# mconati/armour-dev

Hardware: AMD Instinct MI355X
Metric: planning iterations/sec (7-DOF, 100 t-steps, 20 obs) (higher is better)
Workload: dtype f64; 1 GPU; Kinova Gen3 7-DOF, T=100, O=20 box obstacles, 3 concurrent planner(s) x 1308 worlds/GPU/step; obstacles=20, worlds_per_gpu=3924, planners_per_gpu=3, worlds_per_planner=1308, parallelism=world-sharded x1, RCCL all_gather of per-world records

## Files before the change

### armour-dev_amd/armour_amd/__init__.py

```python
from __future__ import annotations

import ctypes
import os

import numpy as np

from .robots import KINOVA
from .worlds import csv_world, example_world, make_world, straight_line_waypoint

_HERE = os.path.dirname(os.path.abspath(__file__))
LIB_PATH = os.environ.get("ARMOUR_LIB") or os.path.join(_HERE, "libarmour_hip.so")
NF = 7
_LIB = None
_dp = ctypes.POINTER(ctypes.c_double)


ARMOUR_E_ARG, ARMOUR_E_HIP, ARMOUR_E_CAPACITY, ARMOUR_E_STATE, ARMOUR_E_INTERNAL = -1, -2, -3, -4, -5


class ArmourError(RuntimeError):
    pass


class Config(ctypes.Structure):
# ... 607 lines not shown
        lk = np.zeros((self.T, self.NJ), dtype=np.int32)
        tq = np.zeros((self.T, NF), dtype=np.int32)
        _check(lib().armour_get_monomial_counts(self.h, w, lk.ctypes.data_as(ctypes.POINTER(ctypes.c_int)),
                                                tq.ctypes.data_as(ctypes.POINTER(ctypes.c_int))))
        return lk, tq

    OCCUPANCY = ("arena_hashes", "arena_rows", "operator_terms", "link_monomials", "torque_monomials",
                 "worlds_retried", "worlds_failed")

    def occupancy(self):
        n = len(self.OCCUPANCY)
        used = (ctypes.c_longlong * n)()
        caps = (ctypes.c_longlong * n)()
        rc = lib().armour_get_reach_occupancy(self.h, used, caps, n)
        _check(min(0, rc))
        return {k: (int(used[i]), int(caps[i])) for i, k in enumerate(self.OCCUPANCY)}

    def reach_span_ms(self):
        v = ctypes.c_double()
        _check(lib().armour_get_reach_span(self.h, ctypes.byref(v)))
        return v.value

    def plane_cache_stats(self):
        keys = ("planes_kept", "pairs", "blocks_cached", "blocks", "max_per_pair", "pool_records", "box_misses")
        out = (ctypes.c_longlong * len(keys))()
        _check(min(0, lib().armour_get_plane_cache_stats(self.h, out, len(keys))))
        return {k: int(out[i]) for i, k in enumerate(keys)}

    def torque_radius(self, w):
        r = np.zeros((self.T, NF))
        _check(lib().armour_get_torque_radius(self.h, w, _ptr(r)))
        return r


def run_episodes(planner, worlds, goals, max_steps, track=None, **config):
    st = planner.episode_begin(worlds, goals, **config)
    if track is not None:
        planner.episode_track(**track)
    running = int(np.sum(st["status"] == 0))
    for _ in range(int(max_steps)):
        if running == 0:
            break
        running, _, _ = planner.episode_step()
    st = planner.episode_states()
    out = dict(status=st["status"], steps=st["steps"], clearance=st["clearance"])
    if track is not None:
        out["tracked"] = planner.episode_tracked()
# ... 39 lines not shown
```

### armour-dev_amd/csrc/nlp.h

```cpp
#pragma once
#include "reach.h"

namespace armour {

constexpr int EVAL_THREADS = 256;
constexpr int ROW_THREADS = 256;
constexpr int MAX_FILTER = 64;
constexpr int KA = 56;
constexpr int KA2 = 8;

struct IpmOpts {
    double tol = 1e-4;
    int max_iter = 100;
    double mu0 = 0.1;
    double kappa_eps = 10.0;
    double kappa_mu = 0.2;
    double theta_mu = 1.5;
    double tau_min = 0.99;
    double bound_push = 1e-2;
    double eta = 1e-4;
    int max_ls = 10;
    double kappa_sigma = 1e10;
    double s_max = 100.0;
    double inf_bound = 1e19;
// ... 56 lines not shown
    WorldState* ws;
    int* flags;
    const int* wl;
    int* wl_run;
    int* wl_search;
    unsigned* cnt;
    int ls0;
    const unsigned* lcount;
    unsigned* lcount_out;
    unsigned* lrun_out;
    int* nrun_flag;
    int* bt_flag;
    int K;
    double *gs, *fs, *partial_s;
    int b_in_cs;
    int resto;
    int rflag;
    int* rl_app;
    int* pend_flag;
    int pcache;
    int pcready;
    long pc_pool;
    double* pc;
    uint16_t* pcp;
    unsigned* pcoff;
    unsigned char* pcok;
    unsigned long long* pcbase;
    unsigned* pcnext;
    const int* Ow;
};
constexpr int EV_MAXK = 9;
constexpr int PC_K = 12;
constexpr double PC_XBOX = 1.0 + 1e-6;
constexpr double PC_RADF = 1.0001;
constexpr double PC_MARGIN = 1e-9;

AD int world_of(const NlpDev& d, int b) { return d.wl ? d.wl[b] : b; }

AD long gidx(const NlpDev& d, int slot, int w, long r) { return ((long)slot * d.W + w) * d.m + r; }

struct Shape {
    int O, m, R, nblk;
};
template <bool MX>
AD Shape shape_of(const NlpDev& d, int w) {
    if constexpr (MX) {
        const int O = d.Ow[w];
        const int m = d.nt + d.T * d.NJ * O + 4 * NF;
        const int R = m + NF;
        return Shape{O, m, R, (R + d.chunk - 1) / d.chunk};
    } else {
        return Shape{d.O, d.m, d.R, d.nblk};
    }
}

// ... 2 lines not shown
```

### armour-dev_amd/csrc/nlp_kernels.hip

```cpp
#include "nlp.h"

namespace armour {

__device__ inline double wave_max(double v) {
#pragma unroll
    for (int m = 1; m < 64; m <<= 1) v = fmax(v, xor_f64(v, m));
    return v;
}
__device__ inline double wave_min(double v) {
#pragma unroll
    for (int m = 1; m < 64; m <<= 1) v = fmin(v, xor_f64(v, m));
    return v;
}
template <int N>
__device__ inline void block_reduce_n(double (&v)[N], const int (&kinds)[N], double* lds, double* out) {
    const int wave = threadIdx.x >> 6, nw = blockDim.x >> 6;
#pragma unroll
    for (int g = 0; g < N; g += 8) {
#pragma unroll
        for (int i = g; i < (g + 8 < N ? g + 8 : N); i++)
            v[i] = kinds[i] == 0 ? wave_sum(v[i]) : kinds[i] == 1 ? wave_max(v[i]) : wave_min(v[i]);
        if ((threadIdx.x & 63) == 0) {
#pragma unroll
            for (int i = g; i < (g + 8 < N ? g + 8 : N); i++) lds[wave * N + i] = v[i];
// ... 346 lines not shown
    const unsigned long long u = __builtin_bit_cast(unsigned long long, x);
    return (u >> 63) ? ~u : (u | 0x8000000000000000ull);
}
__device__ inline double dkey(unsigned long long k) {
    return __builtin_bit_cast(double, (k >> 63) ? (k & 0x7FFFFFFFFFFFFFFFull) : ~k);
}

template <bool MX>
__device__ __attribute__((always_inline)) void plane_cache_body(const NlpDev& d) {
    const int t = blockIdx.x, w = blockIdx.y, tid = threadIdx.x;
    const long jt = (long)w * d.T + t;
    const int NJ = d.NJ, O = shape_of<MX>(d, w).O, NP = NJ * O;
    const int OS = d.O, NPS = NJ * OS;
    __shared__ double cen[MAX_J][3], rad[MAX_J][3];
    __shared__ double lgen[MAX_J][18];
    __shared__ double obs[MAX_OBS][12];
    __shared__ double llp[MAX_J][LL_PLANES][10];
    __shared__ double oop[MAX_OBS][OO_PLANES][5];
    __shared__ double mixlo[MAX_J * MAX_OBS * OBS_GEN];
    __shared__ unsigned char mixbits[MAX_J * MAX_OBS * OBS_GEN];
    __shared__ double pairM[MAX_J * MAX_OBS];
    __shared__ unsigned cntp[MAX_J * MAX_OBS];
    __shared__ unsigned long long pbits[MAX_J * MAX_OBS];
    __shared__ unsigned total_s;
    for (int i = tid; i < NJ * 18; i += blockDim.x) lgen[i / 18][i % 18] = d.ro.link_gens[jt * NJ * 18 + i];
    for (int i = tid; i < O * 12; i += blockDim.x) obs[i / 12][i % 12] = d.obs[(long)w * OS * 12 + i];
    if (tid < NJ * 3) {
        const int l = tid / 3, e = tid % 3;
        const long b = jt * NJ + l;
        const int cnt = d.ro.link_cnt[b];
        double r = 0.0;
        for (int q = 0; q < cnt; q++) r += fabs(d.ro.link_coef[(b * CAP_LM + q) * 3 + e]);
        cen[l][e] = d.ro.link_center[b * 3 + e];
        rad[l][e] = r * PC_RADF;
    }
    __syncthreads();
    for (int u = tid; u < NJ * LL_PLANES + O * OO_PLANES; u += blockDim.x) {
        if (u < NJ * LL_PLANES) ll_table(lgen[u / LL_PLANES], u % LL_PLANES, cen[u / LL_PLANES], llp[u / LL_PLANES][u % LL_PLANES]);
        else oo_table(obs[(u - NJ * LL_PLANES) / OO_PLANES], (u - NJ * LL_PLANES) % OO_PLANES,
                      oop[(u - NJ * LL_PLANES) / OO_PLANES][(u - NJ * LL_PLANES) % OO_PLANES]);
    }
    const int nmix = NP * OBS_GEN;
    auto load_gens = [&](int l, int o, double (*G)[3], double* oc) {
#pragma unroll
        for (int r = 0; r < 3; r++) oc[r] = obs[o][r];
#pragma unroll
        for (int q = 0; q < OBS_GEN; q++)
#pragma unroll
            for (int r = 0; r < 3; r++) G[q][r] = obs[o][(q + 1) * 3 + r];
#pragma unroll
        for (int q = 0; q < 6; q++)
#pragma unroll
            for (int r = 0; r < 3; r++) G[OBS_GEN + q][r] = lgen[l][r + 3 * q];
    };
    __syncthreads();
    for (int u = tid; u < nmix; u += blockDim.x) {
        const int l = u / (O * OBS_GEN), o = (u / OBS_GEN) % O, i = u % OBS_GEN;
        double G[BUF_GEN][3], oc[3];
        load_gens(l, o, G, oc);
        double M = -1e300;
        const double* const ga = obs[o] + 3 * (i + 1);
#pragma unroll
        for (int j = 0; j < 6; j++) {
            double A[3], dd, del, lo, hi;
            mixed_plane_j(j, ga, G, oc, A, dd, del);
            pc_bounds(A, dd + del, -dd + del, cen[l], rad[l], lo, hi);
            if (nonzero3(A)) M = fmax(M, lo);
        }
        mixlo[u] = M;
    }
    __syncthreads();
    for (int pr = tid; pr < NP; pr += blockDim.x) {
        const int l = pr / O, o = pr % O;
        double G[BUF_GEN][3], oc[3];
        load_gens(l, o, G, oc);
        double M = fmax(fmax(mixlo[pr * 3], mixlo[pr * 3 + 1]), mixlo[pr * 3 + 2]);
#pragma unroll
        for (int p = 0; p < OO_PLANES; p++) {
// ... 21 lines not shown
#pragma unroll
        for (int j = 0; j < 6; j++) {
            double A[3], dd, del, lo, hi;
            mixed_plane_j(j, ga, G, oc, A, dd, del);
            pc_bounds(A, dd + del, -dd + del, cen[l], rad[l], lo, hi);
            if (nonzero3(A) && hi >= M) bits |= 1u << j;
        }
        mixbits[u] = (unsigned char)bits;
    }
    __syncthreads();
    auto survives = [&](int pr, int l, int o, int a, int b, const double (*G)[3], const double* oc) -> bool {
        if (a < OBS_GEN && b >= OBS_GEN) return (mixbits[pr * OBS_GEN + a] >> (b - OBS_GEN)) & 1;
        const double* P = b < OBS_GEN ? oop[o][a + b - 1] : llp[l][(a - OBS_GEN) * (11 - (a - OBS_GEN)) / 2 + b - a - 1];
        double dd, del, lo, hi;
        if (b < OBS_GEN) oo_complete(P, G + OBS_GEN, dd, del);
        else ll_complete(P, G, oc, dd, del);
        pc_bounds(P, dd + del, -dd + del, cen[l], rad[l], lo, hi);
        return nonzero3(P) && hi >= pairM[pr] - PC_MARGIN;
    };
    for (int pr = tid; pr < NP; pr += blockDim.x) {
        const int l = pr / O, o = pr % O;
        double G[BUF_GEN][3], oc[3];
        load_gens(l, o, G, oc);
        unsigned n = 0;
        unsigned long long bits = 0;
        int pos = 0;
        for (int a = 0; a < BUF_GEN; a++)
            for (int b = a + 1; b < BUF_GEN; b++, pos++)
                if (survives(pr, l, o, a, b, G, oc)) {
                    n++;
                    bits |= 1ull << pos;
                }
        cntp[pr] = n;
        pbits[pr] = bits;
    }
    __syncthreads();
    if (tid < 64) {
        const int per = (NP + 63) / 64, b0 = tid * per;
        unsigned s = 0;
        for (int q = b0; q < b0 + per && q < NP; q++) s += cntp[q];
        unsigned incl = s;
#pragma unroll
        for (int off = 1; off < 64; off <<= 1) {
            const unsigned v = __shfl_up(incl, off);
            if (tid >= off) incl += v;
        }
        unsigned run = incl - s;
        for (int q = b0; q < b0 + per && q < NP; q++) {
            const unsigned c = cntp[q];
            cntp[q] = run;
            run += c;
            d.pcoff[jt * NPS + q] = (run - c) << 8 | c;
        }
        if (tid == 63) total_s = incl;
    }
    __syncthreads();
    __shared__ unsigned long long base_s;
    if (tid == 0) {
        const unsigned long long b0 = atomicAdd(d.pcnext, total_s);
        const bool fits = b0 + total_s <= (unsigned long long)d.pc_pool;
        d.pcok[jt] = fits ? 1 : 0;
        d.pcbase[jt] = fits ? b0 : 0;
        base_s = fits ? b0 : ~0ull;
    }
    __syncthreads();
    if (base_s == ~0ull) return;
    double* const rec = d.pc + 5 * base_s;
    uint16_t* const pcp = d.pcp + base_s;
    const int cap = (int)total_s;
    for (int pr = tid; pr < NP; pr += blockDim.x) {
        const int l = pr / O, o = pr % O;
        double G[BUF_GEN][3], oc[3];
        load_gens(l, o, G, oc);
        unsigned q = cntp[pr];
        const unsigned long long bits = pbits[pr];
        int pos = 0;
        for (int a = 0; a < BUF_GEN; a++)
            for (int b = a + 1; b < BUF_GEN; b++) {
                if (!((bits >> pos++) & 1ull)) continue;
                double A[3], dd, del;
                if (a < OBS_GEN && b >= OBS_GEN) {
                    mixed_plane_j(b - OBS_GEN, obs[o] + 3 * (a + 1), G, oc, A, dd, del);
                } else {
                    const double* P = b < OBS_GEN ? oop[o][a + b - 1] : llp[l][(a - OBS_GEN) * (11 - (a - OBS_GEN)) / 2 + b - a - 1];
                    A[0] = P[0]; A[1] = P[1]; A[2] = P[2];
                    if (b < OBS_GEN) oo_complete(P, G + OBS_GEN, dd, del);
                    else ll_complete(P, G, oc, dd, del);
                }
                rec[q] = A[0];
                rec[cap + q] = A[1];
                rec[2 * cap + q] = A[2];
                rec[3 * cap + q] = dd + del;
                rec[4 * cap + q] = -dd + del;
                pcp[q] = (uint16_t)pr;
                q++;
            }
    }
}
__global__ __launch_bounds__(EVAL_THREADS) void plane_cache_kernel(NlpDev d) { plane_cache_body<false>(d); }
__global__ __launch_bounds__(EVAL_THREADS) void plane_cache_kernel_mx(NlpDev d) { plane_cache_body<true>(d); }


#define STAGE_MONOMIALS_BODY                                                                        \
    int lpre[MAX_J + 1], tpre[NF + 1];                                                              \
    lpre[0] = 0;                                                                                    \
    _Pragma("unroll") for (int l = 0; l < MAX_J; l++) lpre[l + 1] = lpre[l] + (l < NJ ? lcnt[l] : 0); \
    tpre[0] = 0;                                                                                    \
    _Pragma("unroll") for (int j = 0; j < NF; j++) tpre[j + 1] = tpre[j] + tcnt[j];                 \
    const int L = lpre[MAX_J], M = tpre[NF];                                                        \
    for (int u = threadIdx.x; u < L + M; u += blockDim.x) {                                         \
        if (u < L) {                                                                                \
            int l = 0, q0 = 0;                                                                      \
            _Pragma("unroll") for (int k = 1; k < MAX_J; k++) if (u >= lpre[k]) { l = k; q0 = lpre[k]; } \
            const int q = u - q0;                                                                   \
            const long b = (jt * NJ + l) * CAP_LM + q;                                              \
            lh[l][q] = d.ro.link_hash[b];                                                           \
            lco[l][q][0] = d.ro.link_coef[b * 3];                                                   \
// ... 62 lines not shown
    return r;
}
#define TRAJ_COST_BODY                                                                              \
    for (int j = 0; j < NF; j++)                                                                    \
        qp[j] = bz_q(ts.q0[j], ts.qd0[j] * ts.D, ts.qdd0[j] * ts.D * ts.D, rp.k_range[j] * x[j], tp); \
    double fv = 0.0;                                                                                \
    bool first = true;                                                                              \
    for (int pass = 1; pass >= 0; pass--)                                                           \
        for (int j = 0; j < NF; j++) {                                                              \
            if (rp.wrap_mask[j] != pass) continue;                                                  \
            const double dd = pass ? wrap_to_pi(d.qdes[w * NF + j] - qp[j]) : (d.qdes[w * NF + j] - qp[j]); \
            const double term = dd * dd;                                                            \
            fv = first ? term : fv + term;                                                          \
            first = false;                                                                          \
        }
__device__ __attribute__((always_inline)) double traj_cost(const NlpDev& d, const RobotParams& rp, TrajStart ts, int w,
                                                           const double* x, double* qp) {
    const double tp = rp.t_plan;
    TRAJ_COST_BODY
    return fv;
}

struct PlaneRecords {
    const double* rec;
    const uint16_t* pcp;
    int total;
};
__device__ __attribute__((always_inline)) PlaneRecords plane_records(const NlpDev& d, long jt, int NP, bool some = true) {
    const unsigned last = some ? d.pcoff[jt * (d.NJ * d.O) + NP - 1] : 0u;
    const unsigned long long pb = d.pcbase[jt];
    return {d.pc + 5 * pb, d.pcp + pb, (int)(last >> 8) + (int)(last & 255)};
}
struct PlaneRecord {
    double a[3], P, N;
    int pr;
};
__device__ __attribute__((always_inline)) PlaneRecord load_record(PlaneRecords pc, int q) {
    const int cap = pc.total;
    return {{pc.rec[q], pc.rec[cap + q], pc.rec[2 * cap + q]}, pc.rec[3 * cap + q], pc.rec[4 * cap + q], pc.pcp[q]};
}
__device__ __attribute__((always_inline)) double record_candidate(PlaneRecord r, const double* lc, bool& neg) {
    const double Ac = r.a[0] * lc[0] + r.a[1] * lc[1] + r.a[2] * lc[2];
    const double pos = Ac - r.P, nv = -Ac - r.N;
    neg = nv > pos || pos != pos;
    return neg ? nv : pos;
}
constexpr double SCAN_START = -100000000.0;
__device__ __attribute__((always_inline)) void pair_max(unsigned long long* key, double v) {
    if (v > SCAN_START) atomicMax(key, okey(v));
}

constexpr int UB_FULL = MAX_J * CAP_LM * 3 + NF * CAP_UM;
constexpr int LM_S = 16, UM_S = 64;
constexpr int UB_S = 1544;
static_assert(UB_S >= MAX_J * LM_S * 3 + NF * UM_S, "small staging buffer");
__host__ __device__ constexpr int eval_pair_doubles(int np) { return np + (np + 1) / 2 + 4 * np; }
template <typename R, bool ARMTD, bool CACHED, int LM, int UM, int UB, bool MX = false>
__device__ __attribute__((always_inline)) void eval_body(const NlpDev& d, int mode) {
    static_assert(!CACHED || std::is_same<R, double>::value, "the plane cache is fp64");
    static_assert(!MX || (std::is_same<R, double>::value && !ARMTD), "mixed batches: the fp64 ARMOUR planner");
    if ((mode == 1 || mode == 5) && d.lcount && blockIdx.y >= *d.lcount) return;
    const int t = blockIdx.x, w = world_of(d, blockIdx.y);
    WorldState& S = d.ws[w];
// ... 25 lines not shown
    auto lco = reinterpret_cast<R (*)[LM][3]>(ubuf);
    auto tco = reinterpret_cast<R (*)[UM]>(ubuf + MAX_J * LM * 3);
    constexpr int NMIX = MAX_J * MAX_OBS * OBS_GEN;
    static_assert(CACHED || MAX_J * LL_PLANES * 10 + MAX_OBS * OO_PLANES * 5 + NMIX + (NMIX + 7) / 8 <= UB, "plane tables");
    auto llp = reinterpret_cast<R (*)[LL_PLANES][10]>(ubuf);
    auto oop = reinterpret_cast<R (*)[OO_PLANES][5]>(ubuf + MAX_J * LL_PLANES * 10);
    R* mixv = reinterpret_cast<R*>(ubuf + MAX_J * LL_PLANES * 10 + MAX_OBS * OO_PLANES * 5);
    int8_t* mixc = reinterpret_cast<int8_t*>(mixv + NMIX);
    __shared__ int lcnt[MAX_J], tcnt[NF];
    __shared__ R ptab[NF][8];
    if (tid < NF) {
        const double xd = mode == 0 ? S.x[tid] : S.xt[tid];
        x[tid] = xd;
        const R xj = (R)xd;
        power_table(xj, ptab[tid]);
        ptab[tid][4] = (R)0.0; ptab[tid][5] = (R)1.0 * (R)1.0; ptab[tid][6] = (R)2.0 * xj; ptab[tid][7] = (R)3.0 * (xj * xj);
    }
    if (tid < NJ) lcnt[tid] = d.ro.link_cnt[jt * NJ + tid];
    if (tid >= 32 && tid < 32 + NF) tcnt[tid - 32] = d.nt ? d.ro.tq_cnt[jt * NF + tid - 32] : 0;
    if constexpr (!CACHED) {
        for (int i = tid; i < NJ * 18; i += blockDim.x) lgen[i / 18][i % 18] = d.ro.link_gens[jt * NJ * 18 + i];
        for (int i = tid; i < O * 12; i += blockDim.x) obs[i / 12][i % 12] = d.obs[(long)w * OS * 12 + i];
    }
    __syncthreads();
    EVP_MARK
    if (!(d.diag & 1)) {
        STAGE_MONOMIALS_BODY
    }
    __syncthreads();
    EVP_MARK
    const int nlk = NJ * 3 * 8;
    for (int u = tid; u < ((d.diag & 1) ? 0 : 64 + nlk); u += blockDim.x) {
      if (u >= 64) {
        const int ul = u - 64;
        const int l = ul / 24, e = (ul / 8) % 3, k = ul % 8;
        const long base = jt * NJ + l;
        R c = k == 0 ? d.ro.link_center[base * 3 + e] : 0.0;
        c = sum4(c, lcnt[l], [&](int q) { return slice_term(lco[l][q][e], lh[l][q], k, ptab); });
        if (k == 0) {
            const R r = d.ro.link_rad[base * 3 + e];
            const R cc = interval_mid(c, r);
            lc[l][e] = cc;
            Lcb[((long)t * NJ + l) * 3 + e] = cc;
        } else {
            dlc[l][k - 1][e] = c;
            Jdb[(((long)t * NJ + l) * NF + k - 1) * 3 + e] = c;
// ... 39 lines not shown
            *fb = fv * rp.cost_scale;
            for (int i = 0; i < NF; i++) {
                const double dk = tp * tp * tp * (6 * tp * tp - 15 * tp + 10) * rp.k_range[i];
                double gv = rp.wrap_mask[i] ? (2 * wrap_to_pi(qp[i] - d.qdes[w * NF + i]) * dk) : (2 * (qp[i] - d.qdes[w * NF + i]) * dk);
                gradb[i] = gv * rp.cost_scale;
            }
        }
    }
    __syncthreads();
    EVP_MARK
    const long nt = d.nt;
    bool coll = !(d.diag & 2);
    if constexpr (MX) coll = coll && O > 0;
    if constexpr (CACHED) {
        bool inbox = true;
#pragma unroll
        for (int j = 0; j < NF; j++) inbox = inbox && fabs(x[j]) <= PC_XBOX;
        if (coll && !inbox) {
            for (int pr = tid; pr < NJ * O; pr += blockDim.x)
                Gb[nt + ((long)(pr / O) * d.T + t) * O + pr % O] = __builtin_nan("");
            if (tid == 0) atomicAdd(d.cnt + 7, 1u);
        } else if (coll) {
            const int NP = NJ * O;
            const PlaneRecords pc = plane_records(d, jt, NP);
            const int total = pc.total;
            unsigned long long* const pkey = reinterpret_cast<unsigned long long*>(ubuf);
            unsigned* const pidx = reinterpret_cast<unsigned*>(ubuf + NP);
            double* const pB = ubuf + NP + (NP + 1) / 2;
            static_assert(eval_pair_doubles(MAX_J * MAX_OBS) <= UB_FULL, "pair tables");
            const double start = SCAN_START;
            for (int pr = tid; pr < NP; pr += blockDim.x) {
                pkey[pr] = okey(start);
                pidx[pr] = 0xFFFFFFFFu;
            }
            __syncthreads();
            EVP_MARK
            auto cand = [&](int q, double& v, int& sub, int& pr, double* a) {
                const PlaneRecord r = load_record(pc, q);
                a[0] = r.a[0]; a[1] = r.a[1]; a[2] = r.a[2];
                pr = r.pr;
                bool neg;
                v = record_candidate(r, lc[pr / O], neg);
                sub = neg ? 1 : 0;
            };
            constexpr int RPT = 3;
            if (total <= RPT * EVAL_THREADS) {
                double v[RPT], a[RPT][3];
                int sub[RPT], pq[RPT];
#pragma unroll
                for (int s = 0; s < RPT; s++) {
                    const int q = tid + s * EVAL_THREADS;
                    v[s] = start;
                    sub[s] = 0;
                    pq[s] = 0;
                    if (q < total) {
                        cand(q, v[s], sub[s], pq[s], a[s]);
                        pair_max(&pkey[pq[s]], v[s]);
                    }
                }
                __syncthreads();
                EVP_MARK
#pragma unroll
                for (int s = 0; s < RPT; s++) {
                    const int q = tid + s * EVAL_THREADS;
                    if (q < total && v[s] > start && v[s] == dkey(pkey[pq[s]])) atomicMin(&pidx[pq[s]], (unsigned)(2 * q + sub[s]));
                }
                __syncthreads();
                EVP_MARK
#pragma unroll
                for (int s = 0; s < RPT; s++) {
                    const int q = tid + s * EVAL_THREADS;
                    if (q < total && pidx[pq[s]] == (unsigned)(2 * q + sub[s])) {
                        double* const b = pB + pq[s] * 4;
                        b[0] = a[s][0]; b[1] = a[s][1]; b[2] = a[s][2]; b[3] = v[s];
                    }
                }
            } else {
                for (int q = tid; q < total; q += blockDim.x) {
                    double v, a[3];
                    int sub, pr;
                    cand(q, v, sub, pr, a);
                    pair_max(&pkey[pr], v);
                }
                __syncthreads();
                EVP_MARK
                for (int q = tid; q < total; q += blockDim.x) {
                    double v, a[3];
                    int sub, pr;
                    cand(q, v, sub, pr, a);
                    if (v > start && v == dkey(pkey[pr])) atomicMin(&pidx[pr], (unsigned)(2 * q + sub));
                }
                __syncthreads();
                EVP_MARK
                for (int q = tid; q < total; q += blockDim.x) {
                    double v, a[3];
                    int sub, pr;
                    cand(q, v, sub, pr, a);
                    if (pidx[pr] == (unsigned)(2 * q + sub)) {
                        double* const b = pB + pr * 4;
                        b[0] = a[0]; b[1] = a[1]; b[2] = a[2]; b[3] = v;
                    }
                }
            }
            __syncthreads();
            EVP_MARK
            for (int pr = tid; pr < NP; pr += blockDim.x) {
                const int l = pr / O, o = pr % O;
                const unsigned wi = pidx[pr];
                const bool won = wi != 0xFFFFFFFFu, isneg = won && (wi & 1u);
                const double* const b = pB + pr * 4;
                const double best = won ? b[3] : start;
                const double B0 = won ? b[0] : 0.0, B1 = won ? b[1] : 0.0, B2 = won ? b[2] : 0.0;
                const long row = nt + ((long)l * d.T + t) * O + o;
                Gb[row] = -best;
                double* const jn = Jnb + (row - nt) * 3;
                jn[0] = isneg ? B0 : -B0;
                jn[1] = isneg ? B1 : -B1;
                jn[2] = isneg ? B2 : -B2;
                if (mode == 0) {
#pragma unroll
                    for (int kk = 0; kk < NF; kk++) {
                        const double dot = B0 * dlc[l][kk][0] + B1 * dlc[l][kk][1] + B2 * dlc[l][kk][2];
                        Jb[row * NF + kk] = isneg ? dot : -dot;
                    }
                }
            }
            coll = false;
        }
    }
    if constexpr (!CACHED) {
    for (int u = tid; u < (coll ? NJ * LL_PLANES + O * OO_PLANES : 0); u += blockDim.x) {
        if (u < NJ * LL_PLANES) {
            const int l = u / LL_PLANES, p = u % LL_PLANES;
            ll_table(lgen[l], p, lc[l], llp[l][p]);
        } else {
// ... 193 lines not shown
            const double c = sum4(d.ro.tq_center[base], tcnt[j], [&](int q) { return value_term(tco[j][q], th[j][q], ptab[kk]); });
            d.gs[((long)i * K + kk) * d.m + (long)t * NF + j] = interval_mid(c, d.ro.tq_rad[base]);
        }
    }
    for (int v = t; v <= 2 * NF && tid >= (int)blockDim.x - K; v += d.T) {
        const int kk = tid - ((int)blockDim.x - K);
        const double* x = xk[kk];
        double* const Gb = d.gs + ((long)i * K + kk) * d.m;
        const TrajStart ts = traj_start(d, w);
        if (v < 2 * NF) {
            const long off2 = (long)NF * d.T + (long)d.T * d.NJ * O;
            const int kind = v / NF, j = v % NF;
            const ExtremumRows er = extremum_rows(rp, ts, kind, j, x[j]);
            const long rmin = off2 + kind * 2 * NF + j;
            Gb[rmin] = er.mn;
            Gb[rmin + NF] = er.mx;
            continue;
        }
        double qp[NF];
        d.fs[(long)i * K + kk] = traj_cost(d, rp, ts, w, x, qp) * rp.cost_scale;
    }
    __syncthreads();
    EVP_MARK
    const PlaneRecords pc = plane_records(d, jt, NP, NP > 0);
    unsigned long long* const pkey = reinterpret_cast<unsigned long long*>(ubuf);
    static_assert(EV_MAXK * MAX_J * MAX_OBS <= UB_FULL, "trial pair table");
    for (int u = tid; u < K * NP; u += blockDim.x) pkey[u] = okey(SCAN_START);
    __syncthreads();
    EVP_MARK
    for (int q = tid; q < pc.total; q += blockDim.x) {
        const PlaneRecord r = load_record(pc, q);
        const int l = r.pr / O;
        for (int kk = 0; kk < K; kk++) {
            bool neg;
            pair_max(&pkey[kk * NP + r.pr], record_candidate(r, lck[kk][l], neg));
        }
    }
    __syncthreads();
    EVP_MARK
    for (int u = tid; u < K * NP; u += blockDim.x) {
        const int kk = u / NP, pr = u - kk * NP;
        const int l = pr / O, o = pr % O;
        d.gs[((long)i * K + kk) * d.m + nt + ((long)l * d.T + t) * O + o] = -dkey(pkey[u]);
    }
    EVP_PRINT("TR")
}
__global__ __launch_bounds__(EVAL_THREADS) void eval_trials_kernel(NlpDev d) { eval_trials_body<CAP_LM, CAP_UM, UB_FULL>(d); }
// ... 1418 lines not shown
            const int ul = u - ntv;
            const int kk = ul / (NJ * 3), l = (ul / 3) % NJ, e = ul % 3;
            const long base = jt * NJ + l;
            const double s = sum4(d.ro.link_center[base * 3 + e], lcnt[l],
                                  [&](int q) { return value_term(lco[l][q][e], lh[l][q], ptab[kk]); });
            lck[kk][l][e] = interval_mid(s, d.ro.link_rad[base * 3 + e]);
        } else {
            const int kk = u / NF, j = u % NF;
            const long base = jt * NF + j;
            const double s = sum4(d.ro.tq_center[base], tcnt[j], [&](int q) { return value_term(tco[j][q], th[j][q], ptab[kk]); });
            const double v = interval_mid(s, d.ro.tq_rad[base]);
            const double tr = d.ro.torque_radius[base];
            const double Lb = -rp.torque_limits[j] + tr, Ub = rp.torque_limits[j] - tr;
            const double tv = rp.torque_violation;
            tqv[kk][j] = fmax((Lb - tv) - v, (v - Ub) - tv);
            tqb[kk][j] = (v < Lb - tv || v > Ub + tv) ? 1 : 0;
        }
    }
    __syncthreads();
    {
        const int g = tid >> 6, lane = tid & 63;
        const double cv = rp.collision_violation;
        unsigned long long* const pkey = reinterpret_cast<unsigned long long*>(ubuf);
        const PlaneRecords pc = NP > 0 ? plane_records(d, jt, NP) : PlaneRecords{nullptr, nullptr, 0};
        const int KP = NP > 0 ? min(KC, UB / NP) : KC;
        for (int k0 = 0; k0 < KN; k0 += KP) {
            const int kp = min(KP, KN - k0);
            for (int u = tid; u < kp * NP; u += blockDim.x) pkey[u] = okey(SCAN_START);
            __syncthreads();
            for (int q = tid; q < pc.total; q += blockDim.x) {
                const PlaneRecord r = load_record(pc, q);
                const int pr = min(r.pr, NP - 1), l = pr / O;
                for (int kk = 0; kk < kp; kk++) {
                    bool neg;
                    pair_max(&pkey[kk * NP + pr], record_candidate(r, lck[k0 + kk][l], neg));
                }
            }
            __syncthreads();
            for (int kk = g; kk < kp; kk += EVAL_THREADS / 64) {
                double cm = -__builtin_inf();
                int cb = 0;
                for (int pr = lane; pr < NP; pr += 64) {
                    const double row = -dkey(pkey[kk * NP + pr]);
                    cm = fmax(cm, row - cv);
                    cb |= row > cv ? 1 : 0;
                }
                cm = wave_max(cm);
// ... 104 lines not shown
```

### armour-dev_amd/csrc/planner.hip

```cpp
#include <hip/hip_runtime.h>
#include <chrono>
#include <cmath>
#include <cstdio>
#include <cstdlib>
#include <cstring>
#include <algorithm>
#include <atomic>
#include <string>
#include <vector>

#include "../../include/armour_hip.h"
#include "nlp_kernels.hip"
#include "reach_kernel.hip"
#include "lane_kernel.hip"
#include "motion_kernels.hip"
#include "track_kernels.hip"
#include "robots.h"

using namespace armour;

namespace {
thread_local std::string g_err;

int fail(int code, const std::string& msg) {
// ... 466 lines not shown
    const size_t Rmax = mmax + NF;
    if ((rc = p->alloc(&d.L, Wm * Rmax)) || (rc = p->alloc(&d.U, Wm * Rmax)) || (rc = p->alloc(&d.g, 2 * Wm * mmax)) ||
        (rc = p->alloc(&d.J, 2 * Wm * mmax * NF)) || (rc = p->alloc(&d.f, 2 * (size_t)Wm)) ||
        (rc = p->alloc(&d.grad, 2 * (size_t)Wm * NF)) || (rc = p->alloc(&d.link_c, 3 * jobs * NJ * 3)))
        return rc;
    d.njn = (long)(jobs * NJ * Om * 3);
    d.njd = (long)(jobs * NJ * NF * 3);
    if ((rc = p->alloc(&d.jn, 2 * (size_t)d.njn)) || (rc = p->alloc(&d.jd, 2 * (size_t)d.njd))) return rc;
    double** rowbufs[] = {&d.slo, &d.shi, &d.zlo, &d.zhi, &d.dslo, &d.dshi};
    for (double** b : rowbufs)
        if ((rc = p->alloc(b, Wm * Rmax))) return rc;
    d.chunk = set.row_chunk;
    const int nblk_max = (int)((Rmax + d.chunk - 1) / d.chunk);
    if ((rc = p->alloc(&d.partial, (size_t)Wm * nblk_max * KA)) || (rc = p->alloc(&d.partial2, (size_t)Wm * nblk_max * KA2)) ||
        (rc = p->alloc(&d.ws, (size_t)Wm)) ||
        (rc = p->alloc(&p->feas, (size_t)Wm)))
        return rc;
    HIPCK(hipHostMalloc((void**)&p->h_flags, 12 * sizeof(int), hipHostMallocMapped));
    HIPCK(hipHostGetDevicePointer((void**)&d.flags, p->h_flags, 0));
    if ((rc = p->alloc(&p->d_lists, 6 * (size_t)Wm)) || (rc = p->alloc(&d.cnt, 16))) return rc;
    d.pcache = set.plane_cache && (double)COMB * NJ * std::max(Om, 1) * (double)jobs < 4294967295.0;
    d.pcready = 0;
    d.pc_pool = std::max(1L, (long)std::min(std::max(set.pc_k, 1), COMB) * NJ * std::max(Om, 1) * (long)jobs);
    if (d.pcache && ((rc = p->alloc(&d.pc, 5 * (size_t)d.pc_pool)) || (rc = p->alloc(&d.pcp, (size_t)d.pc_pool)) ||
                     (rc = p->alloc(&d.pcoff, jobs * NJ * (size_t)Om)) || (rc = p->alloc(&d.pcok, jobs)) ||
                     (rc = p->alloc(&d.pcbase, jobs)) || (rc = p->alloc(&d.pcnext, 1))))
        return rc;
    if (d.pcache) {
        HIPCK(hipMemset(d.pcnext, 0, sizeof(unsigned)));
        HIPCK(hipHostMalloc((void**)&p->h_pcnext, sizeof(unsigned)));
        p->rc.pc_next = d.pcnext;
        p->ra.rc.pc_next = d.pcnext;
        p->la.rc.pc_next = d.pcnext;
    }
    d.K = d.opt.max_ls - 1;
    p->spec = !set.no_spec && d.K > 0 && d.K <= EV_MAXK && d.pcache && !p->armtd && !set.eval_f32;
    p->spec_all = p->spec && p->set.tail_search > 0 && (d.K + 1) * NJ * Om <= UB_FULL;
    p->resto_spec = p->spec && d.opt.resto_max > 0 && d.opt.max_ls <= EV_MAXK + 1 && d.opt.max_ls * NJ * Om <= UB_FULL &&
                    !set.resto_rounds;
    p->resto_inline = p->resto_spec && set.resto_inline;
    p->resto_conc = p->resto_inline && p->spec_all && set.tail_worlds > 0 && set.resto_concurrent;
    if (p->resto_conc) {
        HIPCK(hipStreamCreateWithFlags(&p->rstream2, hipStreamNonBlocking));
        HIPCK(hipEventCreateWithFlags(&p->ev_ip, hipEventDisableTiming));
        HIPCK(hipEventCreateWithFlags(&p->ev_pub, hipEventDisableTiming));
        HIPCK(hipEventCreateWithFlags(&p->ev_rend, hipEventDisableTiming));
    }
// ... 280 lines not shown
    p->d.pcready = 0;
    return 0;
}

#define KSEL(k) (p->d.Ow ? k##_mx : k)

static void ensure_plane_cache(armour_planner* p) {
    NlpDev& d = p->d;
    if (!d.pcache || d.pcready || d.O == 0 || p->set.eval_f32) return;
    bool fits = false;
    for (int attempt = 0; attempt < 3; attempt++) {
        hipLaunchKernelGGL(KSEL(plane_cache_kernel), dim3(p->T, p->W), dim3(EVAL_THREADS), 0, p->stream, d);
        if (hipMemcpyAsync(p->h_pcnext, d.pcnext, sizeof(unsigned), hipMemcpyDeviceToHost, p->stream) != hipSuccess ||
            hipStreamSynchronize(p->stream) != hipSuccess)
            break;
        const long need = (long)*p->h_pcnext;
        (void)hipMemsetAsync(d.pcnext, 0, sizeof(unsigned), p->stream);
        if (need <= d.pc_pool) {
            fits = true;
            break;
        }
        if (attempt == 2) break;
        const long grow = need + need / 4;
        double* pc = nullptr;
        uint16_t* pcp = nullptr;
        if (std::getenv("ARMOUR_PC_GROW_FAIL") || dalloc(&pc, 5 * (size_t)grow) != hipSuccess) break;
        if (dalloc(&pcp, (size_t)grow) != hipSuccess) { (void)hipFree(pc); break; }
        for (void*& a : p->allocs) {
            if (a == (void*)d.pc) { (void)hipFree(a); a = pc; }
            else if (a == (void*)d.pcp) { (void)hipFree(a); a = pcp; }
        }
        d.pc = pc;
        d.pcp = pcp;
        d.pc_pool = grow;
    }
    d.pcready = fits ? 1 : 0;
}

static int nside_count(const armour_planner* p) {
    return 2 * p->d.nt + p->T * p->NJ * p->O + 2 * 4 * NF + 2 * NF;
}

static bool eval_small_fits(const armour_planner* p) {
    return !p->set.eval_full && !p->armtd && !p->set.eval_f32 && p->mono_max[0] <= LM_S && p->mono_max[1] <= UM_S;
}
static void launch_eval(armour_planner* p, dim3 grid, const NlpDev& d, int mode, bool cached = true, hipStream_t s = nullptr) {
    if (!s) s = p->stream;
    const bool c = cached && d.pcready && d.O > 0;
    if (c && eval_small_fits(p) && eval_pair_doubles(p->NJ * d.O) <= UB_S) {
        hipLaunchKernelGGL(KSEL(eval_kernel_small), grid, dim3(EVAL_THREADS), 0, s, d, mode);
        return;
    }
    if (d.Ow) {
        hipLaunchKernelGGL(c ? eval_kernel_mx<true> : eval_kernel_mx<false>, grid, dim3(EVAL_THREADS), 0, s, d, mode);
        return;
    }
// ... 1217 lines not shown
        HIPCK(hipMemcpy(link_counts, p->ro.link_cnt + j0 * p->NJ, sizeof(int) * p->T * p->NJ, hipMemcpyDeviceToHost));
    if (torque_counts)
        HIPCK(hipMemcpy(torque_counts, p->ro.tq_cnt + j0 * NF, sizeof(int) * p->T * NF, hipMemcpyDeviceToHost));
    return 0;
}

int armour_get_reach_span(armour_planner* p, double* span_ms) {
    if (!p || !span_ms) return fail(ARMOUR_E_ARG, "null planner or output");
    if (!p->reached) return fail(ARMOUR_E_STATE, "no reach set");
    *span_ms = p->last_span_ms;
    return p->last_span_ms >= 0 ? 0 : fail(ARMOUR_E_STATE, "no device clock span for the last reach");
}

int armour_get_plane_cache_stats(armour_planner* p, long long* out, int n) {
    DeviceScope device_scope(p);
    if (!p) return fail(ARMOUR_E_ARG, "null planner");
    if (!p->reached) return fail(ARMOUR_E_STATE, "no reach set");
    NlpDev& d = p->d;
    if (!d.pcache || p->set.eval_f32 || d.O == 0) return fail(ARMOUR_E_STATE, "plane cache off (ARMOUR_PLANE_CACHE=0, float study or no obstacles)");
    ensure_plane_cache(p);
    const size_t blocks = (size_t)p->W * p->T, NP = (size_t)p->NJ * d.O;
    std::vector<unsigned> off(blocks * NP);
    std::vector<unsigned char> ok(blocks);
    HIPCK(hipMemcpyAsync(off.data(), d.pcoff, sizeof(unsigned) * off.size(), hipMemcpyDeviceToHost, p->stream));
    HIPCK(hipMemcpyAsync(ok.data(), d.pcok, blocks, hipMemcpyDeviceToHost, p->stream));
    HIPCK(hipStreamSynchronize(p->stream));
    long long kept = 0, nok = 0, mx = 0, pairs = 0;
    for (size_t b = 0; b < blocks; b++) {
        const size_t np = (size_t)p->NJ * p->Ow[b / p->T];
        pairs += (long long)np;
        for (size_t q = 0; q < np; q++) {
            const unsigned v = off[b * NP + q];
            kept += v & 255;
            mx = std::max<long long>(mx, v & 255);
        }
    }
    for (unsigned char v : ok) nok += v;
    unsigned miss = 0;
    HIPCK(hipMemcpy(&miss, d.cnt + 7, sizeof(unsigned), hipMemcpyDeviceToHost));
    const long long st[ARMOUR_PC_COUNT] = {kept, pairs, nok, (long long)blocks, mx, d.pc_pool, miss};
    for (int k = 0; k < n && k < ARMOUR_PC_COUNT; k++) out[k] = st[k];
    return ARMOUR_PC_COUNT;
}

int armour_get_reach_occupancy(armour_planner* p, long long* used, long long* caps, int n) {
    DeviceScope device_scope(p);
    if (!p) return fail(ARMOUR_E_ARG, "null planner");
    if (!p->reached) return fail(ARMOUR_E_STATE, "no reach set");
    if (!p->lane_engine || !p->d_occ)
        return fail(ARMOUR_E_STATE, "occupancy is recorded by the bundle engine only (this batch ran on the per-job engine)");
    const unsigned long long* o = p->h_occ;
    const long long u[ARMOUR_OCC_COUNT] = {(long long)o[0], (long long)o[1], (long long)o[2], (long long)o[3],
                                           (long long)o[4], p->last_retried, p->last_failed};
    const long long c[ARMOUR_OCC_COUNT] = {p->la.hcap, p->la.ccap, std::min<long long>(p->la.gcap, (1 << 16) - 1),
                                           CAP_LM, CAP_UM, p->W, p->W};
    for (int k = 0; k < n && k < ARMOUR_OCC_COUNT; k++) {
        if (used) used[k] = u[k];
        if (caps) caps[k] = c[k];
    }
    return ARMOUR_OCC_COUNT;
}

int armour_get_reach_program(const armour_planner* p, int* codes, int capacity) {
// ... 12 lines not shown
```

### include/armour_hip.h

```cpp
#ifndef ARMOUR_HIP_H
#define ARMOUR_HIP_H

#include <stddef.h>

#ifdef __cplusplus
extern "C" {
#endif

#define ARMOUR_NUM_FACTORS 7
#define ARMOUR_OBSTACLE_DOUBLES 12

enum {
    ARMOUR_OK = 0,
    ARMOUR_E_ARG = -1,
    ARMOUR_E_HIP = -2,
    ARMOUR_E_CAPACITY = -3,
    ARMOUR_E_STATE = -4,
    ARMOUR_E_INTERNAL = -5
};

typedef struct armour_planner armour_planner;

typedef struct armour_config {
    int robot;
// ... 178 lines not shown
    double clearance;
    int clearance_at[4];
    double max_pos_err[ARMOUR_NUM_FACTORS], max_vel_err[ARMOUR_NUM_FACTORS], max_torque[ARMOUR_NUM_FACTORS];
    double max_V, max_robust;
    int flags;
    int flag_step[5];
} armour_episode_tracked;
int armour_episode_track(armour_planner* p, const armour_episode_track_config* cfg);
int armour_episode_get_tracked(armour_planner* p, armour_episode_tracked* records, double* true_state, int* flags,
                               double* ms);

int armour_get_constraints(armour_planner* p, int w, double* g);
int armour_get_link_centers(armour_planner* p, int w, double* centers);
int armour_get_link_generators(armour_planner* p, int w, double* gens);
int armour_get_torque_radius(armour_planner* p, int w, double* radius);
int armour_num_joints(const armour_planner* p);
int armour_get_monomial_counts(armour_planner* p, int w, int* link_counts, int* torque_counts);
int armour_get_joint_bounds(const armour_planner* p, double* bounds28);

int armour_get_reach_program(const armour_planner* p, int* codes, int capacity);
#define ARMOUR_OCC_COUNT 7
int armour_get_reach_occupancy(armour_planner* p, long long* used, long long* caps, int n);
int armour_get_reach_profile(armour_planner* p, unsigned long long* cycles_terms, int capacity);
#define ARMOUR_PC_COUNT 7
int armour_get_plane_cache_stats(armour_planner* p, long long* out, int n);
int armour_get_reach_span(armour_planner* p, double* span_ms);
int armour_get_reach_dump(armour_planner* p, double* dump, int capacity);
int armour_sq_selfcheck(int device, double thr, long long half_width, const double* values, long long n,
                        double* s_star, int* valid, long long* mismatches);

#ifdef __cplusplus
}
#endif
#endif
```

Before: 6994 plans/s.

## Compact plane cache records by deduplicating plane normals into shared tables

```diff
diff --git a/armour-dev_amd/armour_amd/__init__.py b/armour-dev_amd/armour_amd/__init__.py
--- a/armour-dev_amd/armour_amd/__init__.py
+++ b/armour-dev_amd/armour_amd/__init__.py
@@ -653,7 +653,8 @@
         return v.value
 
     def plane_cache_stats(self):
-        keys = ("planes_kept", "pairs", "blocks_cached", "blocks", "max_per_pair", "pool_records", "box_misses")
+        keys = ("planes_kept", "pairs", "blocks_cached", "blocks", "max_per_pair", "pool_records", "box_misses",
+                "eval_bytes", "max_per_block")
         out = (ctypes.c_longlong * len(keys))()
         _check(min(0, lib().armour_get_plane_cache_stats(self.h, out, len(keys))))
         return {k: int(out[i]) for i, k in enumerate(keys)}
diff --git a/armour-dev_amd/csrc/nlp.h b/armour-dev_amd/csrc/nlp.h
--- a/armour-dev_amd/csrc/nlp.h
+++ b/armour-dev_amd/csrc/nlp.h
@@ -102,7 +102,10 @@
     int pcready;
     long pc_pool;
     double* pc;
-    uint16_t* pcp;
+    double* pca;
+    unsigned* pcw;
+    double* pcoo;
+    unsigned* pctab;
     unsigned* pcoff;
     unsigned char* pcok;
     unsigned long long* pcbase;
@@ -111,6 +114,10 @@
 };
 constexpr int EV_MAXK = 9;
 constexpr int PC_K = 12;
+constexpr unsigned PC_OO = 0x8000u;
+static_assert(MAX_J * LL_PLANES + MAX_J * MAX_OBS * OBS_GEN * 6 < (int)PC_OO && MAX_OBS * OO_PLANES < (int)PC_OO &&
+                  MAX_J * MAX_OBS <= 0x10000,
+              "a record's word holds the pair in 16 bits and the normal slot in 15");
 constexpr double PC_XBOX = 1.0 + 1e-6;
 constexpr double PC_RADF = 1.0001;
 constexpr double PC_MARGIN = 1e-9;
diff --git a/armour-dev_amd/csrc/nlp_kernels.hip b/armour-dev_amd/csrc/nlp_kernels.hip
--- a/armour-dev_amd/csrc/nlp_kernels.hip
+++ b/armour-dev_amd/csrc/nlp_kernels.hip
@@ -392,7 +392,10 @@
     __shared__ double pairM[MAX_J * MAX_OBS];
     __shared__ unsigned cntp[MAX_J * MAX_OBS];
     __shared__ unsigned long long pbits[MAX_J * MAX_OBS];
-    __shared__ unsigned total_s;
+    __shared__ unsigned cntm[MAX_J * MAX_OBS];
+    __shared__ unsigned llslot[MAX_J * LL_PLANES];
+    __shared__ unsigned total_s, ntab_s;
+    for (int u = tid; u < NJ * LL_PLANES; u += blockDim.x) llslot[u] = 0;
     for (int i = tid; i < NJ * 18; i += blockDim.x) lgen[i / 18][i % 18] = d.ro.link_gens[jt * NJ * 18 + i];
     for (int i = tid; i < O * 12; i += blockDim.x) obs[i / 12][i % 12] = d.obs[(long)w * OS * 12 + i];
     if (tid < NJ * 3) {
@@ -424,6 +427,9 @@
             for (int r = 0; r < 3; r++) G[OBS_GEN + q][r] = lgen[l][r + 3 * q];
     };
     __syncthreads();
+    if (t == 0)
+        for (int u = tid; u < O * OO_PLANES * 3; u += blockDim.x)
+            d.pcoo[(long)w * OS * OO_PLANES * 3 + u] = oop[u / (OO_PLANES * 3)][(u / 3) % OO_PLANES][u % 3];
     for (int u = tid; u < nmix; u += blockDim.x) {
         const int l = u / (O * OBS_GEN), o = (u / OBS_GEN) % O, i = u % OBS_GEN;
         double G[BUF_GEN][3], oc[3];
@@ -491,7 +497,7 @@
         const int l = pr / O, o = pr % O;
         double G[BUF_GEN][3], oc[3];
         load_gens(l, o, G, oc);
-        unsigned n = 0;
+        unsigned n = 0, nm = 0;
         unsigned long long bits = 0;
         int pos = 0;
         for (int a = 0; a < BUF_GEN; a++)
@@ -499,11 +505,39 @@
                 if (survives(pr, l, o, a, b, G, oc)) {
                     n++;
                     bits |= 1ull << pos;
+                    if (a < OBS_GEN && b >= OBS_GEN) nm++;
+                    else if (a >= OBS_GEN) llslot[l * LL_PLANES + (a - OBS_GEN) * (11 - (a - OBS_GEN)) / 2 + b - a - 1] = 1;
                 }
         cntp[pr] = n;
+        cntm[pr] = nm;
         pbits[pr] = bits;
     }
     __syncthreads();
+    if (tid >= 64 && tid < 128) {
+        const int lane = tid - 64;
+        unsigned first = 0;
+        for (int pass = 0; pass < 2; pass++) {
+            unsigned* const c = pass ? cntm : llslot;
+            const int len = pass ? NP : NJ * LL_PLANES;
+            const int per = (len + 63) / 64, b0 = lane * per;
+            unsigned s = 0;
+            for (int q = b0; q < b0 + per && q < len; q++) s += c[q];
+            unsigned incl = s;
+#pragma unroll
+            for (int off = 1; off < 64; off <<= 1) {
+                const unsigned v = __shfl_up(incl, off);
+                if (lane >= off) incl += v;
+            }
+            unsigned run = first + incl - s;
+            for (int q = b0; q < b0 + per && q < len; q++) {
+                const unsigned v = c[q];
+                c[q] = pass == 0 && !v ? 0xFFFFFFFFu : run;
+                run += v;
+            }
+            first += __shfl(incl, 63);
+        }
+        if (lane == 0) ntab_s = first;
+    }
     if (tid < 64) {
         const int per = (NP + 63) / 64, b0 = tid * per;
         unsigned s = 0;
@@ -530,38 +564,48 @@
         const bool fits = b0 + total_s <= (unsigned long long)d.pc_pool;
         d.pcok[jt] = fits ? 1 : 0;
         d.pcbase[jt] = fits ? b0 : 0;
+        d.pctab[jt] = fits ? ntab_s : 0;
         base_s = fits ? b0 : ~0ull;
     }
     __syncthreads();
     if (base_s == ~0ull) return;
-    double* const rec = d.pc + 5 * base_s;
-    uint16_t* const pcp = d.pcp + base_s;
-    const int cap = (int)total_s;
+    double* const pn = d.pc + 2 * base_s;
+    double* const tab = d.pca + 3 * base_s;
+    unsigned* const pcw = d.pcw + base_s;
+    for (int u = tid; u < NJ * LL_PLANES; u += blockDim.x) {
+        const unsigned s = llslot[u];
+        if (s == 0xFFFFFFFFu) continue;
+        const double* P = llp[u / LL_PLANES][u % LL_PLANES];
+        tab[3 * s] = P[0]; tab[3 * s + 1] = P[1]; tab[3 * s + 2] = P[2];
+    }
     for (int pr = tid; pr < NP; pr += blockDim.x) {
         const int l = pr / O, o = pr % O;
         double G[BUF_GEN][3], oc[3];
         load_gens(l, o, G, oc);
-        unsigned q = cntp[pr];
+        unsigned q = cntp[pr], m = cntm[pr];
         const unsigned long long bits = pbits[pr];
         int pos = 0;
         for (int a = 0; a < BUF_GEN; a++)
             for (int b = a + 1; b < BUF_GEN; b++) {
                 if (!((bits >> pos++) & 1ull)) continue;
-                double A[3], dd, del;
+                double dd, del;
+                unsigned ai;
                 if (a < OBS_GEN && b >= OBS_GEN) {
+                    double A[3];
                     mixed_plane_j(b - OBS_GEN, obs[o] + 3 * (a + 1), G, oc, A, dd, del);
+                    tab[3 * m] = A[0]; tab[3 * m + 1] = A[1]; tab[3 * m + 2] = A[2];
+                    ai = m++;
+                } else if (b < OBS_GEN) {
+                    oo_complete(oop[o][a + b - 1], G + OBS_GEN, dd, del);
+                    ai = PC_OO | (unsigned)(o * OO_PLANES + a + b - 1);
                 } else {
-                    const double* P = b < OBS_GEN ? oop[o][a + b - 1] : llp[l][(a - OBS_GEN) * (11 - (a - OBS_GEN)) / 2 + b - a - 1];
-                    A[0] = P[0]; A[1] = P[1]; A[2] = P[2];
-                    if (b < OBS_GEN) oo_complete(P, G + OBS_GEN, dd, del);
-                    else ll_complete(P, G, oc, dd, del);
+                    const int p = (a - OBS_GEN) * (11 - (a - OBS_GEN)) / 2 + b - a - 1;
+                    ll_complete(llp[l][p], G, oc, dd, del);
+                    ai = llslot[l * LL_PLANES + p];
                 }
-                rec[q] = A[0];
-                rec[cap + q] = A[1];
-                rec[2 * cap + q] = A[2];
-                rec[3 * cap + q] = dd + del;
-                rec[4 * cap + q] = -dd + del;
-                pcp[q] = (uint16_t)pr;
+                pn[2 * q] = dd + del;
+                pn[2 * q + 1] = -dd + del;
+                pcw[q] = ai << 16 | (unsigned)pr;
                 q++;
             }
     }
@@ -670,23 +714,29 @@
 }
 
 struct PlaneRecords {
-    const double* rec;
-    const uint16_t* pcp;
+    const double2* pn;
+    const unsigned* pcw;
+    const double* tab;
+    const double* oo;
     int total;
 };
-__device__ __attribute__((always_inline)) PlaneRecords plane_records(const NlpDev& d, long jt, int NP, bool some = true) {
+__device__ __attribute__((always_inline)) PlaneRecords plane_records(const NlpDev& d, int w, long jt, int NP, bool some = true) {
     const unsigned last = some ? d.pcoff[jt * (d.NJ * d.O) + NP - 1] : 0u;
     const unsigned long long pb = d.pcbase[jt];
-    return {d.pc + 5 * pb, d.pcp + pb, (int)(last >> 8) + (int)(last & 255)};
+    return {reinterpret_cast<const double2*>(d.pc) + pb, d.pcw + pb, d.pca + 3 * pb,
+            d.pcoo + (long)w * (d.O * OO_PLANES * 3), (int)(last >> 8) + (int)(last & 255)};
 }
 struct PlaneRecord {
     double a[3], P, N;
     int pr;
 };
-__device__ __attribute__((always_inline)) PlaneRecord load_record(PlaneRecords pc, int q) {
-    const int cap = pc.total;
-    return {{pc.rec[q], pc.rec[cap + q], pc.rec[2 * cap + q]}, pc.rec[3 * cap + q], pc.rec[4 * cap + q], pc.pcp[q]};
-}
+__device__ __attribute__((always_inline)) PlaneRecord load_record(PlaneRecords pc, int q, unsigned wd) {
+    const double2 pn = pc.pn[q];
+    const unsigned s = wd >> 16;
+    const double* const a = ((s & PC_OO) ? pc.oo : pc.tab) + 3 * (s & (PC_OO - 1));
+    return {{a[0], a[1], a[2]}, pn.x, pn.y, (int)(wd & 0xFFFFu)};
+}
+__device__ __attribute__((always_inline)) PlaneRecord load_record(PlaneRecords pc, int q) { return load_record(pc, q, pc.pcw[q]); }
 __device__ __attribute__((always_inline)) double record_candidate(PlaneRecord r, const double* lc, bool& neg) {
     const double Ac = r.a[0] * lc[0] + r.a[1] * lc[1] + r.a[2] * lc[2];
     const double pos = Ac - r.P, nv = -Ac - r.N;
@@ -758,6 +808,15 @@
         for (int i = tid; i < NJ * 18; i += blockDim.x) lgen[i / 18][i % 18] = d.ro.link_gens[jt * NJ * 18 + i];
         for (int i = tid; i < O * 12; i += blockDim.x) obs[i / 12][i % 12] = d.obs[(long)w * OS * 12 + i];
     }
+    constexpr int WPRE = CACHED ? 4 * EVAL_THREADS : 1;
+    __shared__ unsigned wpre[WPRE];
+    PlaneRecords pc{};
+    if constexpr (CACHED) {
+        if (!(d.diag & 2) && O > 0) {
+            pc = plane_records(d, w, jt, NJ * O);
+            for (int q = tid; q < pc.total && q < WPRE; q += blockDim.x) wpre[q] = pc.pcw[q];
+        }
+    }
     __syncthreads();
     EVP_MARK
     if (!(d.diag & 1)) {
@@ -843,11 +902,9 @@
             if (tid == 0) atomicAdd(d.cnt + 7, 1u);
         } else if (coll) {
             const int NP = NJ * O;
-            const PlaneRecords pc = plane_records(d, jt, NP);
             const int total = pc.total;
             unsigned long long* const pkey = reinterpret_cast<unsigned long long*>(ubuf);
             unsigned* const pidx = reinterpret_cast<unsigned*>(ubuf + NP);
-            double* const pB = ubuf + NP + (NP + 1) / 2;
             static_assert(eval_pair_doubles(MAX_J * MAX_OBS) <= UB_FULL, "pair tables");
             const double start = SCAN_START;
             for (int pr = tid; pr < NP; pr += blockDim.x) {
@@ -856,27 +913,28 @@
             }
             __syncthreads();
             EVP_MARK
-            auto cand = [&](int q, double& v, int& sub, int& pr, double* a) {
-                const PlaneRecord r = load_record(pc, q);
-                a[0] = r.a[0]; a[1] = r.a[1]; a[2] = r.a[2];
+            auto record = [&](int q) { return load_record(pc, q, q < WPRE ? wpre[q] : pc.pcw[q]); };
+            auto cand = [&](int q, double& v, int& sub, int& pr) {
+                const PlaneRecord r = record(q);
                 pr = r.pr;
                 bool neg;
                 v = record_candidate(r, lc[pr / O], neg);
                 sub = neg ? 1 : 0;
             };
-            constexpr int RPT = 3;
+            constexpr int RPT = 4;
             if (total <= RPT * EVAL_THREADS) {
-                double v[RPT], a[RPT][3];
-                int sub[RPT], pq[RPT];
+                double v[RPT];
+                int ps[RPT];
 #pragma unroll
                 for (int s = 0; s < RPT; s++) {
                     const int q = tid + s * EVAL_THREADS;
                     v[s] = start;
-                    sub[s] = 0;
-                    pq[s] = 0;
+                    ps[s] = 0;
                     if (q < total) {
-                        cand(q, v[s], sub[s], pq[s], a[s]);
-                        pair_max(&pkey[pq[s]], v[s]);
+                        int sub, pr;
+                        cand(q, v[s], sub, pr);
+                        ps[s] = pr << 1 | sub;
+                        pair_max(&pkey[pr], v[s]);
                     }
                 }
                 __syncthreads();
@@ -884,43 +942,23 @@
 #pragma unroll
                 for (int s = 0; s < RPT; s++) {
                     const int q = tid + s * EVAL_THREADS;
-                    if (q < total && v[s] > start && v[s] == dkey(pkey[pq[s]])) atomicMin(&pidx[pq[s]], (unsigned)(2 * q + sub[s]));
-                }
-                __syncthreads();
-                EVP_MARK
-#pragma unroll
-                for (int s = 0; s < RPT; s++) {
-                    const int q = tid + s * EVAL_THREADS;
-                    if (q < total && pidx[pq[s]] == (unsigned)(2 * q + sub[s])) {
-                        double* const b = pB + pq[s] * 4;
-                        b[0] = a[s][0]; b[1] = a[s][1]; b[2] = a[s][2]; b[3] = v[s];
-                    }
+                    if (q < total && v[s] > start && v[s] == dkey(pkey[ps[s] >> 1]))
+                        atomicMin(&pidx[ps[s] >> 1], (unsigned)(2 * q + (ps[s] & 1)));
                 }
             } else {
                 for (int q = tid; q < total; q += blockDim.x) {
-                    double v, a[3];
+                    double v;
                     int sub, pr;
-                    cand(q, v, sub, pr, a);
+                    cand(q, v, sub, pr);
                     pair_max(&pkey[pr], v);
                 }
                 __syncthreads();
                 EVP_MARK
                 for (int q = tid; q < total; q += blockDim.x) {
-                    double v, a[3];
+                    double v;
                     int sub, pr;
-                    cand(q, v, sub, pr, a);
+                    cand(q, v, sub, pr);
                     if (v > start && v == dkey(pkey[pr])) atomicMin(&pidx[pr], (unsigned)(2 * q + sub));
-                }
-                __syncthreads();
-                EVP_MARK
-                for (int q = tid; q < total; q += blockDim.x) {
-                    double v, a[3];
-                    int sub, pr;
-                    cand(q, v, sub, pr, a);
-                    if (pidx[pr] == (unsigned)(2 * q + sub)) {
-                        double* const b = pB + pr * 4;
-                        b[0] = a[0]; b[1] = a[1]; b[2] = a[2]; b[3] = v;
-                    }
                 }
             }
             __syncthreads();
@@ -929,9 +967,13 @@
                 const int l = pr / O, o = pr % O;
                 const unsigned wi = pidx[pr];
                 const bool won = wi != 0xFFFFFFFFu, isneg = won && (wi & 1u);
-                const double* const b = pB + pr * 4;
-                const double best = won ? b[3] : start;
-                const double B0 = won ? b[0] : 0.0, B1 = won ? b[1] : 0.0, B2 = won ? b[2] : 0.0;
+                double best = start, B0 = 0.0, B1 = 0.0, B2 = 0.0;
+                if (won) {
+                    const PlaneRecord r = record((int)(wi >> 1));
+                    bool neg;
+                    best = record_candidate(r, lc[l], neg);
+                    B0 = r.a[0]; B1 = r.a[1]; B2 = r.a[2];
+                }
                 const long row = nt + ((long)l * d.T + t) * O + o;
                 Gb[row] = -best;
                 double* const jn = Jnb + (row - nt) * 3;
@@ -1171,7 +1213,7 @@
     }
     __syncthreads();
     EVP_MARK
-    const PlaneRecords pc = plane_records(d, jt, NP, NP > 0);
+    const PlaneRecords pc = plane_records(d, w, jt, NP, NP > 0);
     unsigned long long* const pkey = reinterpret_cast<unsigned long long*>(ubuf);
     static_assert(EV_MAXK * MAX_J * MAX_OBS <= UB_FULL, "trial pair table");
     for (int u = tid; u < K * NP; u += blockDim.x) pkey[u] = okey(SCAN_START);
@@ -2636,7 +2678,7 @@
         const int g = tid >> 6, lane = tid & 63;
         const double cv = rp.collision_violation;
         unsigned long long* const pkey = reinterpret_cast<unsigned long long*>(ubuf);
-        const PlaneRecords pc = NP > 0 ? plane_records(d, jt, NP) : PlaneRecords{nullptr, nullptr, 0};
+        const PlaneRecords pc = NP > 0 ? plane_records(d, w, jt, NP) : PlaneRecords{};
         const int KP = NP > 0 ? min(KC, UB / NP) : KC;
         for (int k0 = 0; k0 < KN; k0 += KP) {
             const int kp = min(KP, KN - k0);
diff --git a/armour-dev_amd/csrc/planner.hip b/armour-dev_amd/csrc/planner.hip
--- a/armour-dev_amd/csrc/planner.hip
+++ b/armour-dev_amd/csrc/planner.hip
@@ -512,7 +512,9 @@
     d.pcache = set.plane_cache && (double)COMB * NJ * std::max(Om, 1) * (double)jobs < 4294967295.0;
     d.pcready = 0;
     d.pc_pool = std::max(1L, (long)std::min(std::max(set.pc_k, 1), COMB) * NJ * std::max(Om, 1) * (long)jobs);
-    if (d.pcache && ((rc = p->alloc(&d.pc, 5 * (size_t)d.pc_pool)) || (rc = p->alloc(&d.pcp, (size_t)d.pc_pool)) ||
+    if (d.pcache && ((rc = p->alloc(&d.pc, 2 * (size_t)d.pc_pool)) || (rc = p->alloc(&d.pca, 3 * (size_t)d.pc_pool)) ||
+                     (rc = p->alloc(&d.pcw, (size_t)d.pc_pool)) ||
+                     (rc = p->alloc(&d.pcoo, (size_t)Wm * std::max(Om, 1) * OO_PLANES * 3)) || (rc = p->alloc(&d.pctab, jobs)) ||
                      (rc = p->alloc(&d.pcoff, jobs * NJ * (size_t)Om)) || (rc = p->alloc(&d.pcok, jobs)) ||
                      (rc = p->alloc(&d.pcbase, jobs)) || (rc = p->alloc(&d.pcnext, 1))))
         return rc;
@@ -839,16 +841,19 @@
         }
         if (attempt == 2) break;
         const long grow = need + need / 4;
-        double* pc = nullptr;
-        uint16_t* pcp = nullptr;
-        if (std::getenv("ARMOUR_PC_GROW_FAIL") || dalloc(&pc, 5 * (size_t)grow) != hipSuccess) break;
-        if (dalloc(&pcp, (size_t)grow) != hipSuccess) { (void)hipFree(pc); break; }
+        double *pc = nullptr, *pca = nullptr;
+        unsigned* pcw = nullptr;
+        if (std::getenv("ARMOUR_PC_GROW_FAIL") || dalloc(&pc, 2 * (size_t)grow) != hipSuccess) break;
+        if (dalloc(&pca, 3 * (size_t)grow) != hipSuccess) { (void)hipFree(pc); break; }
+        if (dalloc(&pcw, (size_t)grow) != hipSuccess) { (void)hipFree(pc); (void)hipFree(pca); break; }
         for (void*& a : p->allocs) {
             if (a == (void*)d.pc) { (void)hipFree(a); a = pc; }
-            else if (a == (void*)d.pcp) { (void)hipFree(a); a = pcp; }
+            else if (a == (void*)d.pca) { (void)hipFree(a); a = pca; }
+            else if (a == (void*)d.pcw) { (void)hipFree(a); a = pcw; }
         }
         d.pc = pc;
-        d.pcp = pcp;
+        d.pca = pca;
+        d.pcw = pcw;
         d.pc_pool = grow;
     }
     d.pcready = fits ? 1 : 0;
@@ -2112,23 +2117,30 @@
     const size_t blocks = (size_t)p->W * p->T, NP = (size_t)p->NJ * d.O;
     std::vector<unsigned> off(blocks * NP);
     std::vector<unsigned char> ok(blocks);
+    std::vector<unsigned> tab(blocks);
+    HIPCK(hipMemcpyAsync(tab.data(), d.pctab, sizeof(unsigned) * blocks, hipMemcpyDeviceToHost, p->stream));
     HIPCK(hipMemcpyAsync(off.data(), d.pcoff, sizeof(unsigned) * off.size(), hipMemcpyDeviceToHost, p->stream));
     HIPCK(hipMemcpyAsync(ok.data(), d.pcok, blocks, hipMemcpyDeviceToHost, p->stream));
     HIPCK(hipStreamSynchronize(p->stream));
-    long long kept = 0, nok = 0, mx = 0, pairs = 0;
+    long long kept = 0, nok = 0, mx = 0, pairs = 0, bytes = 0, blk_max = 0;
     for (size_t b = 0; b < blocks; b++) {
         const size_t np = (size_t)p->NJ * p->Ow[b / p->T];
         pairs += (long long)np;
+        long long nb = 0;
         for (size_t q = 0; q < np; q++) {
             const unsigned v = off[b * NP + q];
-            kept += v & 255;
+            nb += v & 255;
             mx = std::max<long long>(mx, v & 255);
         }
+        kept += nb;
+        blk_max = std::max(blk_max, nb);
+        if (ok[b]) bytes += 20 * nb + 24 * (long long)tab[b];
+        if (b % p->T == 0) bytes += 24LL * OO_PLANES * p->Ow[b / p->T];
     }
     for (unsigned char v : ok) nok += v;
     unsigned miss = 0;
     HIPCK(hipMemcpy(&miss, d.cnt + 7, sizeof(unsigned), hipMemcpyDeviceToHost));
-    const long long st[ARMOUR_PC_COUNT] = {kept, pairs, nok, (long long)blocks, mx, d.pc_pool, miss};
+    const long long st[ARMOUR_PC_COUNT] = {kept, pairs, nok, (long long)blocks, mx, d.pc_pool, miss, bytes, blk_max};
     for (int k = 0; k < n && k < ARMOUR_PC_COUNT; k++) out[k] = st[k];
     return ARMOUR_PC_COUNT;
 }
diff --git a/include/armour_hip.h b/include/armour_hip.h
--- a/include/armour_hip.h
+++ b/include/armour_hip.h
@@ -224,7 +224,7 @@
 #define ARMOUR_OCC_COUNT 7
 int armour_get_reach_occupancy(armour_planner* p, long long* used, long long* caps, int n);
 int armour_get_reach_profile(armour_planner* p, unsigned long long* cycles_terms, int capacity);
-#define ARMOUR_PC_COUNT 7
+#define ARMOUR_PC_COUNT 9
 int armour_get_plane_cache_stats(armour_planner* p, long long* out, int n);
 int armour_get_reach_span(armour_planner* p, double* span_ms);
 int armour_get_reach_dump(armour_planner* p, double* dump, int capacity);
```

Result: faster. 7095 plans/s (median of 6 runs) (+1.4%).
